# hermda02/dang

Hardware: AMD Instinct MI355X
Metric: gibbs_iterations_per_sec (higher is better)
Workload: dtype f64

## Files before the change

dang_amd/csrc/dangx_planeset.hip:

```cpp
#ifndef DX_NO_VCOEF
#define DX_VCOEF 1
#endif
#include "dx_host.h"
#include "dx_kern_planeset.h"

static int planeset_jeff(const SweepList& sl) {
    for (int q = 0; q < sl.n; ++q) if (sl.s[q].jeff) return 1;
    return 0;
}
static size_t planeset_lds(int ng, int nb, int nv, int lanes, int Sp, int jeff) {
    const int rows = nv > Sp + jeff ? nv : Sp + jeff;
    return ((size_t)(TROWS * ng + 3) * nb + (size_t)rows * (nb / lanes) * BLOCK) * sizeof(double);
}

static void item_codes(const SweepList& sl, int code[4]) {
    for (int q = 0; q < 4; ++q) code[q] = (q < sl.n) ? sl.s[q].mode + 8 * sl.s[q].pair + 16 * (sl.s[q].jeff ? 1 : 0) : 0;
}
static std::string planeset_name(int Sp, int nb, int ng, int lanes, int solve, const SweepList& sl, int bp) {
    int c[4];
    item_codes(sl, c);
    std::string s = "dxk::k_plane_set<" + std::to_string(Sp) + ", " + std::to_string(nb) + ", " + std::to_string(ng) + ", " + std::to_string(lanes) +
                    ", " + std::to_string(solve);
    for (int q = 0; q < 4; ++q) s += ", " + std::to_string(c[q]);
    return s + ", " + std::to_string(bp) + ">";
}

static int planeset_bp(dangx_ctx* ctx) {
    for (int j = 0; j < ctx->hm.nbands; ++j)
        if (ctx->hm.band[j].n != 0) return 1;
    return 0;
}

static bool planeset_builtin(int nb, int ng, int lanes, int solve, const SweepList& sl) {
    int c[4];
    item_codes(sl, c);
    if (nb == 20 && ng == 6 && lanes == 2) return solve && c[0] == CH_POW && c[1] == CH_MBB_BETA + 8 && c[2] == CH_LOGN_NUP && c[3] == 0;
    if (lanes == 1 && nb == 10 && ng == 4 && solve && sl.n == 0) return true;
    if (lanes == 1 && nb == 10 && ng == 4 && c[0] == CH_POW + 16)
        return c[1] == CH_MBB_BETA + 8 && c[2] == 0 && c[3] == 0;
    if (lanes == 1 && ((nb == 10 && ng == 4) || (solve && ((nb == 5 && ng == 3) || (nb == 3 && ng == 2)))))
        return c[0] == CH_POW && c[1] == CH_MBB_BETA + 8 && c[2] == 0 && c[3] == 0;
    return false;
}

template <int NB, int NG, int LP, int SOLVE, int C0, int C1, int C2>
// ... 39 lines not shown
    return true;
}

int dx_planeset_lanes(dangx_ctx* ctx, const GroupArgs& ga, const SweepList& sl, int solve) {
    static const bool enabled = [] { const char* e = getenv("DANGX_PLANESET"); return !(e && e[0] == '0'); }();
    static const bool small_too = [] { const char* e = getenv("DANGX_PLANESET"); return !(e && e[0] == 'p'); }();
    if (!enabled || sl.n < 0 || sl.n > 4 || (sl.n == 0 && !solve) || ga.ng < 1 || ga.ng > 6) return 0;
    static const int cap2 = [] { const char* e = getenv("DANGX_PS_CAP2"); return e ? atoi(e) : 13; }();
    const int nb = ctx->hm.nbands, Sp = sl.s2 - sl.s1 + 1, cap = (Sp == 2) ? cap2 : 16;
    for (int q = 0; q < sl.n; ++q) {
        const int m = sl.s[q].mode;
        if (m < CH_POW || m > CH_LOGN_W) return 0;
        if (sl.s[q].pair && !(m == CH_MBB_BETA || m == CH_LOGN_NUP)) return 0;
        if (sl.s[q].jeff && m != CH_POW) return 0;
    }
    FusedArgs fa;
    if (!planeset_args(ctx, ga, sl, fa)) return 0;
    if (solve && fa.cal && ga.nuc > 0) return 0;
    const int bp = planeset_bp(ctx), jf = planeset_jeff(sl);
    if (bp) {
        for (int q = 0; q < sl.n; ++q)
            if (sl.s[q].mode > CH_MBB_T || sl.s[q].jeff) return 0;
        if (!(small_too && nb <= cap && planeset_lds(ga.ng, nb, fa.nv, 1, Sp, 0) <= 80u * 1024u)) return 0;
        return dx_rtc_get(ctx, "dx_kern_planeset.h", planeset_name(Sp, nb, ga.ng, 1, solve, sl, 1)) ? 1 : 0;
    }
    int lanes = 0;
    if (small_too && nb <= cap && planeset_lds(ga.ng, nb, fa.nv, 1, Sp, jf) <= 80u * 1024u) lanes = 1;
    else if (nb > 12 && nb % 2 == 0 && nb / 2 <= cap && planeset_lds(ga.ng, nb, fa.nv, 2, Sp, jf) <= 80u * 1024u) lanes = 2;
    if (!lanes) return 0;
    if (planeset_builtin(nb, ga.ng, lanes, solve, sl)) return lanes;
    return dx_rtc_get(ctx, "dx_kern_planeset.h", planeset_name(Sp, nb, ga.ng, lanes, solve, sl, 0)) ? lanes : 0;
}

bool dx_launch_planeset(dangx_ctx* ctx, const GroupArgs& ga, const SweepList& sl, int lanes, int solve, unsigned nblk, unsigned long long* accp) {
    FusedArgs fa;
    if (lanes < 1 || lanes > 2 || !planeset_args(ctx, ga, sl, fa)) return false;
    const int nb = ctx->hm.nbands, ng = ga.ng, Sp = sl.s2 - sl.s1 + 1;
    const size_t ldsz = planeset_lds(ng, nb, fa.nv, lanes, Sp, planeset_jeff(sl));
    const int bp = planeset_bp(ctx);
    if (!bp && planeset_builtin(nb, ng, lanes, solve, sl)) {
        if (planeset_jeff(sl)) dx_launch_planeset_jeff(ctx, ga, fa, sl, Sp, solve, nblk, ldsz, accp);
        else if (nb == 20) launch_builtin<20, 6, 2, 1, CH_POW, CH_MBB_BETA + 8, CH_LOGN_NUP>(ctx, ga, fa, sl, Sp, nblk, ldsz, accp);
        else if (nb == 10 && sl.n == 0) launch_builtin<10, 4, 1, 1, 0, 0, 0>(ctx, ga, fa, sl, Sp, nblk, ldsz, accp);
        else if (nb == 10 && !solve) launch_builtin<10, 4, 1, 0, CH_POW, CH_MBB_BETA + 8, 0>(ctx, ga, fa, sl, Sp, nblk, ldsz, accp);
        else if (nb == 10) launch_builtin<10, 4, 1, 1, CH_POW, CH_MBB_BETA + 8, 0>(ctx, ga, fa, sl, Sp, nblk, ldsz, accp);
        else if (nb == 5) launch_builtin<5, 3, 1, 1, CH_POW, CH_MBB_BETA + 8, 0>(ctx, ga, fa, sl, Sp, nblk, ldsz, accp);
        else launch_builtin<3, 2, 1, 1, CH_POW, CH_MBB_BETA + 8, 0>(ctx, ga, fa, sl, Sp, nblk, ldsz, accp);
        return true;
    }
    hipFunction_t fn = dx_rtc_get(ctx, "dx_kern_planeset.h", planeset_name(Sp, nb, ng, lanes, solve, sl, bp));
    if (!fn) return false;
    const Model* dm = ctx->dm;
    GroupArgs gg = ga;
    SweepList ss = sl;
    unsigned long long* bad = ctx->counters;
    double* part = ctx->partial;
    void* args[] = {&dm, &gg, &fa, &ss, &bad, &accp, &part};
    return dx_rtc_launch(ctx, fn, nblk, ldsz, args) == 0;
}

#endif

#if defined(DX_LNL_DIAG) && !defined(DX_PS_JEFF)
extern "C" int dangx_lnl_diag(unsigned long long* out) {
    if (hipMemcpyFromSymbol(out, HIP_SYMBOL(g_lnl_diag), 2 * sizeof(unsigned long long)) != hipSuccess) return 1;
    const unsigned long long z[2] = {0ull, 0ull};
    return hipMemcpyToSymbol(HIP_SYMBOL(g_lnl_diag), z, sizeof(z)) == hipSuccess ? 0 : 1;
}
#endif
```

dang_amd/csrc/dx_args.h:

```cpp
#pragma once
#include "dx_model.h"
#include "dx_rng.h"
#include "dx_sed.h"

using namespace dx;

constexpr int BLOCK = 256;

struct GroupArgs {
    int ng;
    int gc[MAXG];
    int no;
    int oc[MAXC];
    int flag;
    int ml_mode, fluct;
    unsigned long long seed, stream;
    int nt, nglob;
    int tc[MAXT], trow[MAXT];
    int nuc, uc[MAXC];
};

__device__ __forceinline__ int flag_nplanes(int flag) { return (flag & DANGX_FLAG_QU) ? 2 : 1; }
__device__ __forceinline__ int flag_map(int flag, int p) {
    if (flag & DANGX_FLAG_QU) return 2 + p;
    if (flag & DANGX_FLAG_T) return 1;
    if (flag & DANGX_FLAG_Q) return 2;
    return 3;
}

enum { CH_GENERIC = 0, CH_POW = 1, CH_MBB_BETA = 2, CH_MBB_T = 3, CH_LOGN_NUP = 4, CH_LOGN_W = 5 };

struct IndexArgs {
    int comp, nind, s1, s2, nsample, ml_mode, mode;
    int bp;
    unsigned others;
    int jeff;
    unsigned long long seed, stream;
};

struct SweepItem {
    int comp, nind;
    int mode;
    int pair;
    int gmember;
    int jeff;
    unsigned long long stream, stream2;
};
constexpr int DX_MAX_SWEEPS = 6;
constexpr int DX_MAX_IDXSUM = 8;
struct SweepList {
    int n, nsample, ml_mode, s1, s2, pad;
    unsigned long long seed;
    SweepItem s[DX_MAX_SWEEPS];
};
```

dang_amd/csrc/dx_chain.h:

```cpp
#pragma once
#include "dx_args.h"


template <bool V> struct BoolTag { static constexpr bool value = V; };

#ifdef DX_CHAIN_LIBEXP
#define CEXP(x) exp(x)
#define CEXPS(x) exp(x)
#define CEXP1(x) exp(x)
#else
#define CEXP(x) exp_nr(x)
#define CEXPS(x) exp_sat(x)
#define CEXP1(x) exp_nr_v(x)
#endif
#ifdef DX_CHAIN_IEEEDIV
#define CDIV(a, b) ((a) / (b))
#else
#define CDIV(a, b) ((a) * fast_rcp(b))
#endif

#ifndef DX_CHAIN_UNSCALED
#define DX_CHAIN_SCALED 1
#endif
#ifndef DX_CHAIN_PAIR_RNG
// ... 18 lines not shown
}

__device__ __forceinline__ bool mh_certain(double dlo, double dhi, double u3, bool& acc) {
    const float uf = (float)u3;
    const float elo = __builtin_amdgcn_exp2f((float)dlo * 0x1.715476p+0f);
    const float ehi = __builtin_amdgcn_exp2f((float)dhi * 0x1.715476p+0f);
    acc = (dlo >= 0.0) || (elo > uf * 0x1.001p+0f);
    return acc || ((dhi < 0.0) && (ehi < uf * 0x1.ffep-1f));
}


#ifdef DX_LNL_DIAG
__device__ unsigned long long g_lnl_diag[2];
__device__ __forceinline__ void lnl_diag_count(int k) {
    if (__lane_id() == __builtin_ctzll(__builtin_amdgcn_ballot_w64(true))) atomicAdd(&g_lnl_diag[k], 1ull);
}
#endif

template <int LP>
struct BandPick {
    int half;
    __device__ __forceinline__ double operator()(const double* arr, int j, int nbh) const {
        if (LP == 1) return arr[j];
        const double a = arr[j], b = arr[nbh + j];
        return half ? b : a;
    }
    __device__ __forceinline__ double nu_c(const Model& M, int j, int nbh) const {
        if (LP == 1) return M.band[j].nu_c;
        const double a = M.band[j].nu_c, b = M.band[nbh + j].nu_c;
        return half ? b : a;
    }
};

template <int MODE, int SP, int NB, int LP, bool KT = false, bool BP = false, bool JF = false>
struct RegChain {
    static constexpr bool kBP = BP;
    static constexpr bool kJF = JF;
    static_assert(!JF || (MODE == CH_POW && !BP), "Jeffreys chains: power law, delta bands");
    double D[SP][NB], F[NB], ISr[SP][NB];
    double bpa, bpb;
    double K1[(LP > 1 && !KT) ? NB : 1], K2[(LP > 1 && !KT) ? NB : 1];
    const double *kt1, *kt2;
    double amp[SP];
    double W[(JF && !KT) ? NB : 1], jS;
    double* wcol;

    __device__ __forceinline__ double w(int j) const { return KT ? wcol[j * BLOCK] : W[j]; }
    template <class ISF>
    __device__ __forceinline__ void form_w(const Model& M, const Comp& c, ISF is_of) {
        bool bad = false;
#pragma unroll
        for (int kk = 0; kk < SP; ++kk) bad = bad || !(fabs(amp[kk]) > 0.0 && fabs(amp[kk]) < INFINITY);
#pragma unroll
        for (int j = 0; j < NB; ++j) {
            const double t0 = is_of(0, j) * is_of(0, j);
            double q = t0 * t0;
            if (SP == 2) { const double t1 = is_of(SP - 1, j) * is_of(SP - 1, j); q = fma(t1, t1, q); }
            const double l = k1(M, c, j);
            const double wj = bad ? __longlong_as_double(0x7ff8000000000000ll) : (l * l) * q;
            if (KT) wcol[j * BLOCK] = wj; else W[j] = wj;
        }
    }
    __device__ __forceinline__ void jeff_eval(const Model& M, const Comp& c, double th) {
        double S = 0.0;
#pragma unroll
        for (int j = 0; j < NB; ++j) { const double e = CEXP(th * k1(M, c, j)); S = fma(e * e, w(j), S); }
        if (LP > 1) S += __shfl_xor(S, 1, 64);
        jS = S;
    }

    __device__ __forceinline__ double is(int kk, int j) const { return ISr[kk][j]; }
    __device__ __forceinline__ void set_is(int kk, int j, double v) { ISr[kk][j] = v; }
    __device__ __forceinline__ double k1(const Model& M, const Comp& c, int j) const {
        if (KT) return kt1[j];
        if (LP > 1) return K1[j];
        return (MODE == CH_MBB_T) ? M.band[j].nu_c : (MODE == CH_LOGN_NUP) ? c.lnu9[j] : c.lnr[j];
    }
    __device__ __forceinline__ double k2(const Comp& c, int j) const { return KT ? kt2[j] : (LP > 1) ? K2[j] : c.cst[j]; }
    __device__ __forceinline__ void set_kt(const double* tab, int nbands, int ng, int g, int jb) {
        kt1 = tab + ((MODE == CH_MBB_T) ? TROWS * ng : (MODE == CH_LOGN_NUP) ? TROWS * g + 2 : TROWS * g) * nbands + jb;
        kt2 = tab + (TROWS * g + 1) * nbands + jb;
    }
    __device__ __forceinline__ void set_k(const Model& M, const Comp& c, const BandPick<LP>& pick) {
        if (LP > 1 && !KT) {
#pragma unroll
            for (int j = 0; j < NB; ++j) {
                K1[j] = (MODE == CH_MBB_T) ? pick.nu_c(M, j, NB) : (MODE == CH_LOGN_NUP) ? pick(c.lnu9, j, NB) : pick(c.lnr, j, NB);
                K2[j] = (MODE == CH_LOGN_NUP || MODE == CH_LOGN_W) ? pick(c.cst, j, NB) : 0.0;
            }
        }
    }

    template <bool BATCH, int OP = 0>
    __device__ __forceinline__ double lnl(const Model& M, const Comp& c, double th, double other, double& acc0, double& acc1) {
        double s0 = 0.0, s1 = 0.0;
        if (MODE == CH_POW) s0 = th;
        else if (MODE == CH_MBB_BETA) s0 = th + 1.0;
        else if (MODE == CH_MBB_T) { s0 = mbb_z(th); s1 = CEXP(s0 * c.nu_ref) - 1.0; }
        else if (MODE == CH_LOGN_NUP) { s0 = log_pos(th); s1 = other; }
        else s1 = th;
        acc0 = 0.0; acc1 = 0.0;
        double S = 0.0;
#ifdef DX_CHAIN_IEEEDIV
        const double rs1 = 1.0 / s1;
#else
        const double rs1 = (MODE == CH_LOGN_NUP || MODE == CH_LOGN_W) ? fast_rcp(s1) : 0.0;
#endif
        constexpr int TT = BP ? 1 : (NB % 5 == 0) ? 5 : (NB % 4 == 0) ? 4 : (NB % 3 == 0) ? 3 : 1;
        static_assert(!BP || (LP == 1 && (MODE == CH_POW || MODE == CH_MBB_BETA || MODE == CH_MBB_T)), "bandpass chains: one lane, power law / mbb");
#pragma unroll
        for (int j0 = 0; j0 < NB; j0 += TT) {
            double s[TT];
            if (BP && M.band[j0].n != 0) {
                const Band& b = M.band[j0];
                const kptr nu = as_const(M.bp_nu0 + b.off);
                const kptr tau = as_const(M.bp_tau0 + b.off);
                const kptr lnr = as_const(c.bp_lnr + b.off);
                const int n = b.n;
                double sj = 0.0;
                if (MODE == CH_POW) {
#pragma unroll 4
                    for (int q = 0; q < n; ++q) sj = sj + tau[q] * CEXP(s0 * lnr[q]);
                } else if (MODE == CH_MBB_BETA) {
#pragma unroll 4
                    for (int q = 0; q < n; ++q) sj = sj + (tau[q] * bpb) * fast_rcp(CEXP(bpa * nu[q]) - 1.0) * CEXP(s0 * lnr[q]);
                } else {
#pragma unroll 4
                    for (int q = 0; q < n; ++q) sj = sj + (tau[q] * s1) * fast_rcp(CEXP(s0 * nu[q]) - 1.0) * CEXP(bpa * lnr[q]);
                }
                s[0] = sj;
            } else
            if (MODE == CH_MBB_T && TT > 1 && BATCH) {
                double den[TT], pre[TT];
#pragma unroll
                for (int t = 0; t < TT; ++t) den[t] = CEXP(s0 * k1(M, c, j0 + t)) - 1.0;
                pre[0] = den[0];
#pragma unroll
                for (int t = 1; t < TT; ++t) pre[t] = pre[t - 1] * den[t];
                double inv = s1 * fast_rcp(pre[TT - 1]);
#pragma unroll
                for (int t = TT - 1; t > 0; --t) {
                    s[t] = (inv * pre[t - 1]) * F[j0 + t];
                    inv *= den[t];
                }
                s[0] = inv * F[j0];
            } else
#pragma unroll
            for (int t = 0; t < TT; ++t) {
                const int j = j0 + t;
                if (MODE == CH_LOGN_NUP) {
                    const double l = (k1(M, c, j) - s0) * rs1;
                    s[t] = CEXPS(-0.5 * (l * l)) * k2(c, j);
                } else if (MODE == CH_LOGN_W) {
                    const double l = F[j] * rs1;
                    s[t] = CEXPS(-0.5 * (l * l)) * k2(c, j);
                } else {
                    const double e = CEXP(s0 * k1(M, c, j));
                    if (MODE == CH_POW) s[t] = e;
                    else if (MODE == CH_MBB_BETA) s[t] = F[j] * e;
                    else s[t] = CDIV(s1, e - 1.0) * F[j];
                }
            }
#pragma unroll
            for (int t = 0; t < TT; ++t) {
                const int j = j0 + t;
#ifdef DX_CHAIN_SCALED
                if (OP == 1) {
                    const double r0 = D[0][j];
                    D[0][j] = fma(is(0, j), s[t], r0);
                    acc0 = fma(r0, r0, acc0);
                    if (SP == 2) {
                        const double r1 = D[SP - 1][j];
                        D[SP - 1][j] = fma(is(SP - 1, j), s[t], r1);
                        acc1 = fma(r1, r1, acc1);
                    }
                } else if (OP == 2) {
                    const double r0 = fma(-is(0, j), s[t], D[0][j]);
                    D[0][j] = r0;
                    acc0 = fma(r0, r0, acc0);
                    if (SP == 2) {
                        const double r1 = fma(-is(SP - 1, j), s[t], D[SP - 1][j]);
                        D[SP - 1][j] = r1;
                        acc1 = fma(r1, r1, acc1);
                    }
                } else {
                const double r0 = fma(-is(0, j), s[t], D[0][j]);
                acc0 = fma(r0, r0, acc0);
                if (SP == 2) {
                    const double r1 = fma(-is(SP - 1, j), s[t], D[SP - 1][j]);
                    acc1 = fma(r1, r1, acc1);
                }
                }
                if (JF && OP != 2) S = fma(s[t] * s[t], w(j), S);
#else
                const double r0 = (D[0][j] - amp[0] * s[t]) * is(0, j);
                acc0 = acc0 - 0.5 * (r0 * r0);
                if (SP == 2) {
                    const double r1 = (D[SP - 1][j] - amp[SP - 1] * s[t]) * is(SP - 1, j);
                    acc1 = acc1 - 0.5 * (r1 * r1);
                }
#endif
            }
        }
        if (LP > 1) {
            acc0 += __shfl_xor(acc0, 1, 64);
            if (SP == 2) acc1 += __shfl_xor(acc1, 1, 64);
            if (JF && OP != 2) S += __shfl_xor(S, 1, 64);
        }
        if (JF && OP != 2) jS = S;
#ifdef DX_CHAIN_SCALED
        acc0 *= -0.5; acc1 *= -0.5;
#endif
        return acc0 + acc1;
    }

    __device__ __forceinline__ double lnl_cheap(const Model& M, const Comp& c, double th) {
        double s0 = 0.0, s1 = 0.0;
        if (MODE == CH_POW) s0 = th;
        else if (MODE == CH_MBB_BETA) s0 = th + 1.0;
        else { s0 = mbb_z(th); s1 = CEXP(s0 * c.nu_ref) - 1.0; }
        const double s0l = s0 * 0x1.71547652b82fep+0;
        double acc0 = 0.0, acc1 = 0.0;
#pragma unroll
        for (int j = 0; j < NB; ++j) {
            const float e = __builtin_amdgcn_exp2f((float)(s0l * k1(M, c, j)));
            double s;
            if (MODE == CH_POW) s = (double)e;
            else if (MODE == CH_MBB_BETA) s = F[j] * (double)e;
            else s = (s1 * F[j]) * (double)__builtin_amdgcn_rcpf(e - 1.0f);
            const double r0 = fma(-is(0, j), s, D[0][j]);
            acc0 = fma(r0, r0, acc0);
            if (SP == 2) {
                const double r1 = fma(-is(SP - 1, j), s, D[SP - 1][j]);
                acc1 = fma(r1, r1, acc1);
            }
        }
        double a = acc0 + acc1;
        if (LP > 1) a += __shfl_xor(a, 1, 64);
        return a;
    }

    __device__ __forceinline__ bool cheap_bound(const Model& M, const Comp& c, double lo, double hi, double a_start,
                                                double& wA, double& wG) {
        double G = 0.0, emax = 0.0, kmax = 0.0;
        double smax, zmin = 0.0;
        if (MODE == CH_POW) smax = fmax(fabs(lo), fabs(hi));
        else if (MODE == CH_MBB_BETA) smax = fmax(fabs(lo + 1.0), fabs(hi + 1.0));
        else { smax = mbb_z(lo); zmin = mbb_z(hi); }
// ... 74 lines not shown
        for (int j = 0; j < NB; ++j) { const double s = CEXP(pr.p0 * pick(c2.lnr, j, NB)); Da[j] -= ampa * s; Db[j] -= ampb * s; }
        break;
    case DANGX_MBB:
#pragma unroll
        for (int j = 0; j < NB; ++j) {
            const double s = CDIV(pr.p2, CEXP(pr.p1 * pick.nu_c(M, j, NB)) - 1.0) * CEXP(pr.p0 * pick(c2.lnr, j, NB));
            Da[j] -= ampa * s; Db[j] -= ampb * s;
        }
        break;
    case DANGX_FREEFREE:
#pragma unroll
        for (int j = 0; j < NB; ++j) {
            const double s = ff_gaunt(pick(c2.lnu9, j, NB), pr.p0) / pr.p1 * pick(c2.cst, j, NB);
            Da[j] -= ampa * s; Db[j] -= ampb * s;
        }
        break;
    case DANGX_LOGNORMAL: {
        const double rp1 = fast_rcp(pr.p1);
#pragma unroll
        for (int j = 0; j < NB; ++j) {
            const double l2 = (pick(c2.lnu9, j, NB) - pr.p2) * rp1;
            const double s = CEXPS(-0.5 * (l2 * l2)) * pick(c2.cst, j, NB);
            Da[j] -= ampa * s; Db[j] -= ampb * s;
        }
        break;
    }
    default:
#pragma unroll
        for (int j = 0; j < NB; ++j) { const double s = pick(c2.cst, j, NB); Da[j] -= ampa * s; Db[j] -= ampb * s; }
        break;
    }
}

template <int MODE, int SP, int NB, int LP, bool SCALE = true, bool ADD = false, bool SUB = false, class RC>
__device__ __forceinline__ unsigned long long chain_finish(const Model& M, const IndexArgs& a, const Comp& c, RC& R,
                                                           const BandPick<LP>& pick, double sample0, double sample1, int i, int half,
                                                           double chi[4], double* final_value = nullptr,
                                                           const double* acc_in = nullptr, double* acc_out = nullptr) {
    const int npix = M.npix;
    double* out = c.idx + ((long long)a.nind * M.nmaps) * npix + i;
    const bool first = (a.nind == 0);
    constexpr bool JEFF = RC::kJF;
#if !defined(DX_CHAIN_SCALED)
    static_assert(!JEFF, "the Jeffreys chain exists in the scaled form");
#endif
    if (JEFF && SCALE) R.form_w(M, c, [&](int kk, int j) { return R.is(kk, j); });
    if (SCALE) R.scale();
    if (MODE == CH_MBB_BETA) {
        const double z = mbb_z(sample1);
        const double A = CEXP(z * c.nu_ref) - 1.0;
#pragma unroll
        for (int j = 0; j < NB; ++j) R.F[j] = CDIV(A, CEXP(z * pick.nu_c(M, j, NB)) - 1.0);
        if (RC::kBP) { R.bpa = z; R.bpb = A; }
    } else if (MODE == CH_MBB_T) {
#pragma unroll
        for (int j = 0; j < NB; ++j) R.F[j] = CEXP((sample0 + 1.0) * pick(c.lnr, j, NB));
        if (RC::kBP) R.bpa = sample0 + 1.0;
    } else if (MODE == CH_LOGN_W) {
        {
            const double lp = log_pos(sample0);
#pragma unroll
            for (int j = 0; j < NB; ++j) R.F[j] = pick(c.lnu9, j, NB) - lp;
        }
    }
    const double other = first ? sample1 : sample0;
    const unsigned long long gpix = (unsigned long long)(M.pix0 + i);
    const int q = a.nind;
    const bool gauss = c.prior_type[q] == DANGX_PRIOR_GAUSSIAN;
    const double pmean = c.gauss[q][0], pstd = c.gauss[q][1], lgden = c.lgden[q];
    const double inv2v = 1.0 / (2 * (pstd * pstd));
    auto prior = [&](double v) -> double {
        if (!gauss) return 0.0;
#ifdef DX_CHAIN_IEEEDIV
        const double arg = ((v - pmean) * (v - pmean)) / (2 * (pstd * pstd));
#else
        const double arg = ((v - pmean) * (v - pmean)) * inv2v;
#endif
        return (arg > 745.0) ? -INFINITY : -arg - lgden;
    };
    auto jprior = [&](double S) -> double {
        double p = log_pos(sqrt(S));
        if (!(S >= 0x1p-1022 && S < INFINITY)) p = log(sqrt(S));
        return p;
    };
    unsigned long long nacc = 0;
    double cur = first ? sample0 : sample1;
    double a0, a1, c0, c1;
    const double step = c.step[q], lo = c.uni[q][0], hi = c.uni[q][1];
    const bool ml_opt = (a.ml_mode == DANGX_ML_OPTIMIZE);
#if defined(DX_LNL_EXACT) || !defined(DX_CHAIN_SCALED)
    constexpr bool kCert = false;
#else
    constexpr bool kCert = !RC::kBP && !JEFF && (MODE == CH_POW || MODE == CH_MBB_BETA || MODE == CH_MBB_T);
#endif
    auto chain = [&](auto batch_tag) {
        constexpr bool B = decltype(batch_tag)::value;
        double lnl;
        if (acc_in) { a0 = acc_in[0]; a1 = acc_in[1]; lnl = a0 + a1; if (JEFF) R.jeff_eval(M, c, cur); }
        else lnl = R.template lnl<B, ADD ? 1 : 0>(M, c, cur, other, a0, a1);
        chi[0] = -2.0 * a0; chi[1] = -2.0 * a1;
        double lnl_old = lnl + (JEFF ? jprior(R.jS) : prior(cur));
        bool cert = false, old_exact = true, sums_exact = true;
        double wA = 0.0, wG = 0.0, wold = 0.0;
        if (kCert) {
            const bool ok = R.cheap_bound(M, c, lo, hi, -2.0 * lnl, wA, wG) && !ml_opt;
            cert = __builtin_amdgcn_ballot_w64(!ok) == 0ull;
        }
        auto mh_step = [&](double prop, double u3) {
            if (prop < lo || prop > hi) return;
            if constexpr (!kCert) {
                lnl = R.template lnl<B>(M, c, prop, other, c0, c1);
                const double lnl_new = lnl + (JEFF ? jprior(R.jS) : prior(prop));
                const double diff = lnl_new - lnl_old;
                const bool acc = ml_opt ? (diff > 0.0) : mh_accept(diff, u3);
                if (acc) { cur = prop; lnl_old = lnl_new; a0 = c0; a1 = c1; ++nacc; }
            } else {
                const double pp = prior(prop);
                bool acc = false, und = true;
                double lc = 0.0, wc = 0.0;
                if (cert) {
                    const double A = R.lnl_cheap(M, c, prop);
                    lc = -0.5 * A;
                    wc = fma(wA, A, wG);
                    const double dc = (lc + pp) - lnl_old;
                    const double W = (wc + wold) * (1.0 + 0x1p-40) + 0x1p-49 * ((fabs(lc) + fabs(pp)) + fabs(lnl_old));
                    und = !mh_certain(dc - W, dc + W, u3, acc);
#ifdef DX_LNL_DIAG
                    lnl_diag_count(0);
                    if (__builtin_amdgcn_ballot_w64(und) != 0ull) lnl_diag_count(1);
#endif
                }
// ... 9 lines not shown
                        }
                        const double lnl_new = lnl + pp;
                        const double diff = lnl_new - lnl_old;
                        acc = ml_opt ? (diff > 0.0) : mh_accept(diff, u3);
                        if (acc) { lnl_old = lnl_new; a0 = c0; a1 = c1; }
                        old_exact = true;
                        wold = 0.0;
                    }
                }
                if (acc) {
                    cur = prop;
                    ++nacc;
                    sums_exact = und;
                    if (!und) { lnl_old = lc + pp; wold = wc; old_exact = false; }
                }
            }
        };
        if (LP == 1 || DX_CHAIN_PAIR_RNG == 0) {
            for (int l = 1; l <= a.nsample; ++l) {
                double u1, u2, u3;
                uniform3(a.seed, a.stream, gpix, (uint32_t)l, u1, u2, u3);
                mh_step(cur + rand_normal(0.0, step, u1, u2), u3);
            }
        } else {
            for (int l = 1; l <= a.nsample; l += 2) {
                double u1, u2, u3;
                uniform3(a.seed, a.stream, gpix, (uint32_t)(l + half), u1, u2, u3);
                const double g = rand_normal(0.0, step, u1, u2);
                const double go = __shfl_xor(g, 1, 64), uo = __shfl_xor(u3, 1, 64);
                mh_step(cur + (half == 0 ? g : go), half == 0 ? u3 : uo);
                if (l + 1 <= a.nsample) mh_step(cur + (half == 0 ? go : g), half == 0 ? uo : u3);
            }
        }
        if (SUB) {
            double s0_, s1_;
            (void)R.template lnl<B, 2>(M, c, cur, other, s0_, s1_);
            if (!sums_exact) { a0 = s0_; a1 = s1_; }
        } else if (kCert) {
            if (__builtin_amdgcn_ballot_w64(!sums_exact) != 0ull) {
                if (!sums_exact) (void)R.template lnl<B>(M, c, cur, other, a0, a1);
            }
        }
    };
#ifdef DX_CHAIN_NO_BATCH_RCP
    chain(BoolTag<false>{});
#else
    if (MODE == CH_MBB_T && !RC::kBP) {
        const double tmin = fmin(lo, cur);
#ifdef DX_BATCH_ALWAYS
        chain(BoolTag<true>{});
#elif defined(DX_BATCH_LANEWISE)
        if (tmin > 0.0 && mbb_z(tmin) * M.mbb_batch_z < 1.0) chain(BoolTag<true>{});
        else chain(BoolTag<false>{});
#else
        const bool unsafe = !(tmin > 0.0 && mbb_z(tmin) * M.mbb_batch_z < 1.0);
        if (__builtin_amdgcn_ballot_w64(unsafe) == 0ull) chain(BoolTag<true>{});
        else chain(BoolTag<false>{});
#endif
    } else {
        chain(BoolTag<false>{});
    }
#endif
    if (final_value) *final_value = cur;
    if (acc_out) { acc_out[0] = a0; acc_out[1] = a1; }
    if (half != 0) {
        chi[0] = chi[1] = 0.0;
        return 0ull;
    }
#pragma unroll
// ... 121 lines not shown
```

dang_amd/csrc/dx_kern_fused.h:

```cpp
#pragma once
#include "dx_chain.h"

struct FusedArgs {
    signed char vslot[MAXG];
    signed char vcomp[MAXG];
    signed char vtype[MAXG];
    int nv;
    int gself;
    int cal;
};

#ifndef DX_FUSED_WAVES
#define DX_FUSED_WAVES(SP, NB) 2
#endif
#ifndef DX_FUSED_GRP
#define DX_FUSED_GRP 5
#endif
namespace dxk {

template <int NBL>
__device__ __forceinline__ void sed_column(int type, const double* __restrict__ tab, int NB, int NG, int g, int jb, const Prep& p,
                                           double* __restrict__ colg) {
    const double* lnr = tab + (TROWS * g) * NB + jb;
    const double* cst = lnr + NB;
    const double* lnu9 = cst + NB;
    const double* nuc = tab + (TROWS * NG) * NB + jb;
    constexpr int TT = (NBL % 5 == 0) ? 5 : (NBL % 4 == 0) ? 4 : (NBL % 3 == 0) ? 3 : 1;
    if (type == DANGX_POWERLAW) {
#pragma unroll 1
        for (int j0 = 0; j0 < NBL; j0 += TT) {
#pragma unroll
            for (int t = 0; t < TT; ++t) colg[(j0 + t) * BLOCK] = exp_nr(p.p0 * lnr[j0 + t]);
        }
    } else if (type == DANGX_MBB) {
#pragma unroll 1
        for (int j0 = 0; j0 < NBL; j0 += TT) {
            double f[TT];
#pragma unroll
            for (int t = 0; t < TT; ++t) f[t] = p.p2 * fast_rcp(exp_nr(p.p1 * nuc[j0 + t]) - 1.0);
            __builtin_amdgcn_sched_barrier(0);
#pragma unroll
            for (int t = 0; t < TT; ++t) colg[(j0 + t) * BLOCK] = f[t] * exp_nr(p.p0 * lnr[j0 + t]);
        }
    } else if (type == DANGX_FREEFREE) {
        const double rp1 = fast_rcp(p.p1);
#pragma unroll 1
        for (int j0 = 0; j0 < NBL; j0 += TT) {
#pragma unroll
            for (int t = 0; t < TT; ++t) colg[(j0 + t) * BLOCK] = (ff_gaunt(lnu9[j0 + t], p.p0) * rp1) * cst[j0 + t];
        }
    } else {
        const double rp1 = fast_rcp(p.p1);
#pragma unroll 1
        for (int j0 = 0; j0 < NBL; j0 += TT) {
#pragma unroll
            for (int t = 0; t < TT; ++t) {
                const double l = (lnu9[j0 + t] - p.p2) * rp1;
                colg[(j0 + t) * BLOCK] = exp_sat(-0.5 * (l * l)) * cst[j0 + t];
            }
        }
    }
}

template <int NBL>
__device__ __forceinline__ void sed_column_bp(const Model& M, const Comp& c2, const double* __restrict__ tab, int NB, int NG, int g,
                                              const Prep& p, double* __restrict__ colg) {
#pragma unroll 1
    for (int j = 0; j < NBL; ++j) colg[j * BLOCK] = (M.band[j].n != 0) ? sed_bandpass(M, c2, j, p) : sed_eval_tab(c2.type, tab, NB, NG, g, j, p);
}

template <int MODE, int SP, int NB, int NG, int LP, bool JF = false>
__global__ __launch_bounds__(BLOCK, DX_FUSED_WAVES(SP, NB)) void k_amp_index(const Model* __restrict__ Mp, GroupArgs ga, FusedArgs fa, IndexArgs a,
// ... 198 lines not shown
```

dang_amd/csrc/dx_kern_planeset.h:

```cpp
#pragma once
#include "dx_kern_fused.h"

#ifndef DX_PS_WAVES
#define DX_PS_WAVES(SP, NB, LP, SOLVE, C0) (((NB) / (LP) <= 5) ? 3 : 2)
#endif

namespace dxk {

template <int V> struct ItemCode { static constexpr int value = V; };
template <bool V> struct ItemFlag { static constexpr bool value = V; };

template <int MODE, int PAIR, int SP, int NBL, int LP, int NG, bool FIRST, bool LAST, bool BP, bool JF, typename RFirst>
__device__ __forceinline__ void ps_item(const Model& M, const SweepList& sl, const SweepItem& it, RFirst& R0, int i, int half,
                                        int jb, int NB, const double* __restrict__ tab, const double* __restrict__ col,
                                        double& sample0, double& sample1, double chi_first[4],
                                        double chi_last[4], unsigned int* __restrict__ accepted, int slot, const double* first_acc,
                                        double* wrow) {
    const Comp& c = M.comp[it.comp];
    const BandPick<LP> pick = {half};
    const int npix = M.npix;
    IndexArgs a;
    a.comp = it.comp; a.nind = it.nind; a.s1 = sl.s1; a.s2 = sl.s2; a.nsample = sl.nsample; a.ml_mode = sl.ml_mode; a.mode = MODE;
    a.bp = 0; a.others = 0u; a.jeff = 0; a.seed = sl.seed; a.stream = it.stream;
    RegChain<MODE, SP, NBL, LP, true, BP, JF> R;
    R.set_kt(tab, NB, NG, it.gmember, jb);
#pragma unroll
    for (int kk = 0; kk < SP; ++kk) {
        R.amp[kk] = c.amp[(long long)(sl.s1 + kk - 1) * npix + i];
#pragma unroll
        for (int j = 0; j < NBL; ++j) { R.D[kk][j] = R0.D[kk][j]; R.ISr[kk][j] = col[(kk * NBL + j) * BLOCK] * R.amp[kk]; }
    }
    if (JF) {
        R.wcol = wrow;
        R.form_w(M, c, [&](int kk, int j) { return col[(kk * NBL + j) * BLOCK]; });
    }
    double chia[4] = {0.0, 0.0, 0.0, 0.0}, va, acc[2];
    unsigned long long na = chain_finish<MODE, SP, NBL, LP, false, !FIRST, (!PAIR && !LAST)>(M, a, c, R, pick, sample0, sample1, i, half, chia, &va,
                                                                                            FIRST ? first_acc : nullptr, acc);
    if (it.nind == 0) sample0 = va; else sample1 = va;
    if (FIRST) { chi_first[0] = chia[0]; chi_first[1] = chia[1]; }
    chi_last[2] = chia[2]; chi_last[3] = chia[3];
    unsigned long long nb_ = 0ull;
    if (PAIR) {
        constexpr int MODEB = (MODE == CH_MBB_BETA || MODE == CH_LOGN_NUP) ? MODE + 1 : MODE;
        RegChain<MODEB, SP, NBL, LP, true, BP> RB;
        RB.set_kt(tab, NB, NG, it.gmember, jb);
#pragma unroll
        for (int kk = 0; kk < SP; ++kk) {
            RB.amp[kk] = R.amp[kk];
#pragma unroll
            for (int j = 0; j < NBL; ++j) { RB.D[kk][j] = R.D[kk][j]; RB.ISr[kk][j] = R.ISr[kk][j]; }
        }
        IndexArgs b = a;
        b.nind = it.nind + 1; b.stream = it.stream2; b.mode = MODEB;
        double chib[4] = {0.0, 0.0, 0.0, 0.0}, vb;
        nb_ = chain_finish<MODEB, SP, NBL, LP, false, false, !LAST>(M, b, c, RB, pick, sample0, sample1, i, half, chib, &vb, acc);
        if (b.nind == 0) sample0 = vb; else sample1 = vb;
        chi_last[2] = chib[2]; chi_last[3] = chib[3];
        if (!LAST) {
#pragma unroll
            for (int kk = 0; kk < SP; ++kk)
#pragma unroll
                for (int j = 0; j < NBL; ++j) R0.D[kk][j] = RB.D[kk][j];
        }
    } else if (!LAST) {
#pragma unroll
        for (int kk = 0; kk < SP; ++kk)
#pragma unroll
            for (int j = 0; j < NBL; ++j) R0.D[kk][j] = R.D[kk][j];
    }
    if (accepted) {
        const int copy = threadIdx.x & 15;
        if (na) atomicAdd(accepted + (slot << 4) + copy, (unsigned int)na);
        if (nb_) atomicAdd(accepted + ((slot + 1) << 4) + copy, (unsigned int)nb_);
    }
}

template <int SP, int NB, int NG, int LP, int SOLVE, int C0, int C1, int C2, int C3, int BP = 0>
__global__ __launch_bounds__(BLOCK, DX_PS_WAVES(SP, NB, LP, SOLVE, C0)) void k_plane_set(const Model* __restrict__ Mp, GroupArgs ga, FusedArgs fa, SweepList sl,
// ... 3 lines not shown
    extern __shared__ double lds[];
    const Model& M = *Mp;
    const int npix = M.npix, tid = threadIdx.x;
    double* tab = lds;
    double* col = lds + (TROWS * NG + 3) * NB + tid;
    const long long t0 = (long long)blockIdx.x * BLOCK + tid;
    const long long u = t0 / LP;
    const int half = (int)(t0 % LP), jb = half * NBL;
    const bool in_range = u < npix;
    const int i = in_range ? (int)u : 0;
    const double mk = M.mask[i];
    sed_table_build(M, tab, tid, BLOCK, ga.gc, NG);
    __shared__ unsigned int acc_blk[DX_MAX_IDXSUM * 16];
    if (tid < DX_MAX_IDXSUM * 16) acc_blk[tid] = 0u;
    __syncthreads();
    double chi[4] = {0.0, 0.0, 0.0, 0.0};
    constexpr int NS0 = C0 ? 1 + ((C0 >> 3) & 1) : 0, NS1 = C1 ? 1 + ((C1 >> 3) & 1) : 0, NS2 = C2 ? 1 + ((C2 >> 3) & 1) : 0, NS3 = C3 ? 1 + ((C3 >> 3) & 1) : 0;
    constexpr int NS = NS0 + NS1 + NS2 + NS3;
    const bool live = in_range && !is_masked(mk);
    if (in_range && !live && half == 0) {
        for (int q = 0; q < sl.n; ++q) {
            const Comp& c = M.comp[sl.s[q].comp];
            for (int e = 0; e <= sl.s[q].pair; ++e) {
                double* out = c.idx + ((long long)(sl.s[q].nind + e) * M.nmaps) * npix + i;
#pragma unroll
                for (int kk = 0; kk < SP; ++kk) out[(long long)(sl.s1 + kk - 1) * npix] = 0.0;
            }
        }
    }
    if (live) {
        const long long bstride = (long long)M.nmaps * npix;
        const unsigned long long gpix = (unsigned long long)(M.pix0 + i);
        const bool sample = (ga.ml_mode == DANGX_ML_SAMPLE);
#pragma unroll 1
        for (int v = 0; v < fa.nv; ++v) {
            const Comp& c2 = M.comp[ga.gc[fa.vcomp[v]]];
            double t0v, t1v;
            load_theta(M, c2, i, sl.s1, t0v, t1v);
            if (BP) sed_column_bp<NBL>(M, c2, tab, NB, NG, fa.vcomp[v], sed_prep(c2, t0v, t1v), col + (v * NBL) * BLOCK);
            else sed_column<NBL>(fa.vtype[v], tab, NB, NG, fa.vcomp[v], jb, sed_prep(c2, t0v, t1v), col + (v * NBL) * BLOCK);
        }
        RegChain<CH_POW, SP, NBL, LP> R0;
#pragma unroll
        for (int kk = 0; kk < SP; ++kk) {
            const int k = sl.s1 + kk;
            {
                const double* sigp = M.sig + (long long)(k - 1) * npix + i;
                const double* rmsp = M.rms + (long long)(k - 1) * npix + i;
#pragma unroll
                for (int j = 0; j < NBL; ++j) { R0.D[kk][j] = sigp[(jb + j) * bstride]; R0.ISr[kk][j] = rmsp[(jb + j) * bstride]; }
            }
            auto cal_transform = [&]() {
                const double* gn = tab + (TROWS * NG + 1) * NB + jb;
#pragma unroll
                for (int j = 0; j < NBL; ++j) R0.D[kk][j] = (R0.D[kk][j] - gn[NB + j]) / gn[j];
            };
            if (!SOLVE && SP == 1 && fa.cal) cal_transform();
#pragma unroll 1
            for (int t = 0; t < ga.nuc; ++t) {
                const Comp& ct = M.comp[ga.uc[t]];
                const double tv = ct.tmpl[(long long)(k - 1) * npix + i];
#pragma unroll
                for (int j = 0; j < NBL; ++j) R0.D[kk][j] -= ct.tamp[k - 1][jb + j] * tv;
            }
            double bv[NG];
            if (SOLVE) {
                double eta = 0.0, f0 = 0.0;
                if (sample) {
                    double u1, u2;
                    uniform2(ga.seed, ga.stream, gpix, (uint32_t)k, u1, u2);
                    eta = rand_normal(0.0, 1.0, u1, u2);
                }
                double A[NG * (NG + 1) / 2];
// ... 118 lines not shown
                const double* m = col + (fa.vslot[it0.gmember] * NBL) * BLOCK;
#pragma unroll
                for (int kk = 0; kk < SP; ++kk) {
                    const double a0 = M.comp[it0.comp].amp[(long long)(sl.s1 + kk - 1) * npix + i];
                    double acc = 0.0;
#pragma unroll
                    for (int j = 0; j < NBL; ++j) {
                        const double r = R0.D[kk][j];
                        acc = fma(r, r, acc);
                        R0.D[kk][j] = fma(a0 * R0.ISr[kk][j], m[j * BLOCK], r);
                    }
                    if (LP > 1) acc += __shfl_xor(acc, 1, 64);
                    first_acc[kk] = -0.5 * acc;
                }
            }
#pragma unroll
            for (int kk = 0; kk < SP; ++kk)
#pragma unroll
                for (int j = 0; j < NBL; ++j) col[(kk * NBL + j) * BLOCK] = R0.ISr[kk][j];
            __builtin_amdgcn_sched_barrier(0);
        }
        int slot = 0;
        auto run = [&](auto code_tag, auto first_tag, auto last_tag, int q) {
            constexpr int CODE = decltype(code_tag)::value;
            constexpr bool FIRST = decltype(first_tag)::value;
            constexpr bool LAST = decltype(last_tag)::value;
            if constexpr (CODE != 0) {
                const SweepItem it = sl.s[q];
                const Comp& c = M.comp[it.comp];
                double sample0, sample1, unused[4];
                load_theta(M, c, i, sl.s1, sample0, sample1);
                ps_item<(CODE & 7), ((CODE >> 3) & 1), SP, NBL, LP, NG, FIRST, LAST, (BP != 0), ((CODE >> 4) != 0)>(M, sl, it, R0, i, half, jb, NB, tab, col, sample0, sample1,
                                                                              FIRST ? chi : unused, chi, accepted ? acc_blk : nullptr, slot, first_acc,
                                                                              col + (SP * NBL) * BLOCK);
                slot += 1 + ((CODE >> 3) & 1);
            }
        };
        run(ItemCode<C0>{}, ItemFlag<true>{}, ItemFlag<C1 == 0>{}, 0);
        run(ItemCode<C1>{}, ItemFlag<false>{}, ItemFlag<C2 == 0>{}, 1);
        run(ItemCode<C2>{}, ItemFlag<false>{}, ItemFlag<C3 == 0>{}, 2);
        run(ItemCode<C3>{}, ItemFlag<false>{}, ItemFlag<true>{}, 3);
    }
    if (accepted && NS > 0) {
        __syncthreads();
        if (tid < NS) {
            unsigned int v = 0u;
            for (int q = 0; q < 16; ++q) v += acc_blk[(tid << 4) + q];
            if (v != 0u) atomicAdd(accepted + tid, (unsigned long long)v);
        }
    }
    if (chi_partial) {
        double isum[NS > 0 ? NS : 1];
#pragma unroll
        for (int q = 0; q < (NS > 0 ? NS : 1); ++q) isum[q] = 0.0;
        if (live && half == 0) {
            constexpr int code[4] = {C0, C1, C2, C3};
            constexpr int first[4] = {0, NS0, NS0 + NS1, NS0 + NS1 + NS2};
#pragma unroll
            for (int q = 0; q < 4; ++q)
                if (code[q] != 0) {
                    const double* at = M.comp[sl.s[q].comp].idx + ((long long)sl.s[q].nind * M.nmaps + (sl.s1 - 1)) * npix + i;
                    isum[first[q]] = at[0];
                    if (((code[q] >> 3) & 1) != 0) isum[first[q] + 1] = at[(long long)M.nmaps * npix];
                }
        }
        __shared__ double sh[4 + NS][BLOCK / 64];
#pragma unroll
// ... 16 lines not shown
```

Measured before the change: 98.80.

## Keep MBB factors from SED pass and hand exp terms between paired chains

While building the SED columns, the MBB Planck factor for the beta-sweep component is now stored in an extra LDS row, and the beta chain reads it instead of recomputing exp terms. When the chain is not first, its starting lnL is formed by adding the cached column rather than re-evaluating. At the end of the beta chain, the per-band exponentials are exported and handed to the paired temperature chain as its F factor, which skips a recompute. This costs one more LDS row per block and adds new template paths. These paths can be disabled with DX_BOUNDARY_REEVAL.

```diff
diff --git a/dang_amd/csrc/dangx_planeset.hip b/dang_amd/csrc/dangx_planeset.hip
--- a/dang_amd/csrc/dangx_planeset.hip
+++ b/dang_amd/csrc/dangx_planeset.hip
@@ -8,9 +8,25 @@
     for (int q = 0; q < sl.n; ++q) if (sl.s[q].jeff) return 1;
     return 0;
 }
-static size_t planeset_lds(int ng, int nb, int nv, int lanes, int Sp, int jeff) {
-    const int rows = nv > Sp + jeff ? nv : Sp + jeff;
+static size_t planeset_lds(int ng, int nb, int nv, int lanes, int Sp, int jeff, int keep = 0) {
+    const int rows = (nv > Sp + jeff ? nv : Sp + jeff) + (keep ? 1 : 0);
     return ((size_t)(TROWS * ng + 3) * nb + (size_t)rows * (nb / lanes) * BLOCK) * sizeof(double);
+}
+
+static int planeset_keep(const SweepList& sl, const FusedArgs& fa, int ng, int nb, int lanes, int Sp, int bp) {
+#ifdef DX_BOUNDARY_REEVAL
+    return 0;
+#else
+    if (lanes != 1 || bp || planeset_jeff(sl)) return 0;
+    const int n = sl.n < 4 ? sl.n : 4;
+    for (int q = 0; q < n; ++q) {
+        if (sl.s[q].mode != CH_MBB_BETA) continue;
+        const int v = fa.vslot[sl.s[q].gmember];
+        if (v < 0 || planeset_lds(ng, nb, fa.nv, lanes, Sp, 0, 1) > 80u * 1024u) return 0;
+        return (q > 0 && v >= Sp) ? 2 : 1;
+    }
+    return 0;
+#endif
 }
 
 static void item_codes(const SweepList& sl, int code[4]) {
@@ -116,12 +132,14 @@
     return dx_rtc_get(ctx, "dx_kern_planeset.h", planeset_name(Sp, nb, ga.ng, lanes, solve, sl, 0)) ? lanes : 0;
 }
 
-bool dx_launch_planeset(dangx_ctx* ctx, const GroupArgs& ga, const SweepList& sl, int lanes, int solve, unsigned nblk, unsigned long long* accp) {
+bool dx_launch_planeset(dangx_ctx* ctx, const GroupArgs& ga, const SweepList& sl_in, int lanes, int solve, unsigned nblk, unsigned long long* accp) {
     FusedArgs fa;
-    if (lanes < 1 || lanes > 2 || !planeset_args(ctx, ga, sl, fa)) return false;
+    if (lanes < 1 || lanes > 2 || !planeset_args(ctx, ga, sl_in, fa)) return false;
+    SweepList sl = sl_in;
     const int nb = ctx->hm.nbands, ng = ga.ng, Sp = sl.s2 - sl.s1 + 1;
-    const size_t ldsz = planeset_lds(ng, nb, fa.nv, lanes, Sp, planeset_jeff(sl));
     const int bp = planeset_bp(ctx);
+    sl.keep = planeset_keep(sl, fa, ng, nb, lanes, Sp, bp);
+    const size_t ldsz = planeset_lds(ng, nb, fa.nv, lanes, Sp, planeset_jeff(sl), sl.keep);
     if (!bp && planeset_builtin(nb, ng, lanes, solve, sl)) {
         if (planeset_jeff(sl)) dx_launch_planeset_jeff(ctx, ga, fa, sl, Sp, solve, nblk, ldsz, accp);
         else if (nb == 20) launch_builtin<20, 6, 2, 1, CH_POW, CH_MBB_BETA + 8, CH_LOGN_NUP>(ctx, ga, fa, sl, Sp, nblk, ldsz, accp);
diff --git a/dang_amd/csrc/dx_args.h b/dang_amd/csrc/dx_args.h
--- a/dang_amd/csrc/dx_args.h
+++ b/dang_amd/csrc/dx_args.h
@@ -49,7 +49,8 @@
 constexpr int DX_MAX_SWEEPS = 6;
 constexpr int DX_MAX_IDXSUM = 8;
 struct SweepList {
-    int n, nsample, ml_mode, s1, s2, pad;
+    int n, nsample, ml_mode, s1, s2;
+    int keep;
     unsigned long long seed;
     SweepItem s[DX_MAX_SWEEPS];
 };
diff --git a/dang_amd/csrc/dx_chain.h b/dang_amd/csrc/dx_chain.h
--- a/dang_amd/csrc/dx_chain.h
+++ b/dang_amd/csrc/dx_chain.h
@@ -74,10 +74,12 @@
     }
 };
 
-template <int MODE, int SP, int NB, int LP, bool KT = false, bool BP = false, bool JF = false>
+template <int MODE, int SP, int NB, int LP, bool KT = false, bool BP = false, bool JF = false, bool KEPT = false>
 struct RegChain {
     static constexpr bool kBP = BP;
     static constexpr bool kJF = JF;
+    static constexpr bool kKept = KEPT;
+    static_assert(!KEPT || (LP == 1 && !BP && !JF && (MODE == CH_MBB_BETA || MODE == CH_MBB_T)), "kept factors: one-lane delta-band mbb chains");
     static_assert(!JF || (MODE == CH_POW && !BP), "Jeffreys chains: power law, delta bands");
     double D[SP][NB], F[NB], ISr[SP][NB];
     double bpa, bpb;
@@ -86,6 +88,7 @@
     double amp[SP];
     double W[(JF && !KT) ? NB : 1], jS;
     double* wcol;
+    const double* fcol;
 
     __device__ __forceinline__ double w(int j) const { return KT ? wcol[j * BLOCK] : W[j]; }
     template <class ISF>
@@ -133,8 +136,10 @@
         }
     }
 
-    template <bool BATCH, int OP = 0>
-    __device__ __forceinline__ double lnl(const Model& M, const Comp& c, double th, double other, double& acc0, double& acc1) {
+    template <bool BATCH, int OP = 0, bool EOUT = false>
+    __device__ __forceinline__ double lnl(const Model& M, const Comp& c, double th, double other, double& acc0, double& acc1,
+                                          double* eout = nullptr) {
+        static_assert(!EOUT || (MODE == CH_MBB_BETA && !BP), "the exported factor is the beta chain's");
         double s0 = 0.0, s1 = 0.0;
         if (MODE == CH_POW) s0 = th;
         else if (MODE == CH_MBB_BETA) s0 = th + 1.0;
@@ -198,6 +203,7 @@
                     s[t] = CEXPS(-0.5 * (l * l)) * k2(c, j);
                 } else {
                     const double e = CEXP(s0 * k1(M, c, j));
+                    if (EOUT) eout[j] = e;
                     if (MODE == CH_POW) s[t] = e;
                     else if (MODE == CH_MBB_BETA) s[t] = F[j] * e;
                     else s[t] = CDIV(s1, e - 1.0) * F[j];
@@ -256,6 +262,25 @@
         return acc0 + acc1;
     }
 
+    __device__ __forceinline__ double lnl_add_kept(const double* scol, double& acc0, double& acc1) {
+        static_assert(LP == 1 && !JF && !BP, "one lane, delta bands, no prior sum");
+        acc0 = 0.0; acc1 = 0.0;
+#pragma unroll
+        for (int j = 0; j < NB; ++j) {
+            const double s = scol[j * BLOCK];
+            const double r0 = D[0][j];
+            D[0][j] = fma(is(0, j), s, r0);
+            acc0 = fma(r0, r0, acc0);
+            if (SP == 2) {
+                const double r1 = D[SP - 1][j];
+                D[SP - 1][j] = fma(is(SP - 1, j), s, r1);
+                acc1 = fma(r1, r1, acc1);
+            }
+        }
+        acc0 *= -0.5; acc1 *= -0.5;
+        return acc0 + acc1;
+    }
+
     __device__ __forceinline__ double lnl_cheap(const Model& M, const Comp& c, double th) {
         double s0 = 0.0, s1 = 0.0;
         if (MODE == CH_POW) s0 = th;
@@ -396,11 +421,13 @@
     }
 }
 
-template <int MODE, int SP, int NB, int LP, bool SCALE = true, bool ADD = false, bool SUB = false, class RC>
+template <int MODE, int SP, int NB, int LP, bool SCALE = true, bool ADD = false, bool SUB = false, bool HAND = false, class RC>
 __device__ __forceinline__ unsigned long long chain_finish(const Model& M, const IndexArgs& a, const Comp& c, RC& R,
                                                            const BandPick<LP>& pick, double sample0, double sample1, int i, int half,
                                                            double chi[4], double* final_value = nullptr,
-                                                           const double* acc_in = nullptr, double* acc_out = nullptr) {
+                                                           const double* acc_in = nullptr, double* acc_out = nullptr,
+                                                           double* hand = nullptr, const double* scol = nullptr) {
+    static_assert(!HAND || (MODE == CH_MBB_BETA && !SUB && !RC::kBP && LP == 1), "the hand-over is the one-lane delta-band beta chain's");
     const int npix = M.npix;
     double* out = c.idx + ((long long)a.nind * M.nmaps) * npix + i;
     const bool first = (a.nind == 0);
@@ -410,7 +437,11 @@
 #endif
     if (JEFF && SCALE) R.form_w(M, c, [&](int kk, int j) { return R.is(kk, j); });
     if (SCALE) R.scale();
-    if (MODE == CH_MBB_BETA) {
+    if (MODE == CH_MBB_BETA && RC::kKept && R.fcol) {
+#pragma unroll
+        for (int j = 0; j < NB; ++j) R.F[j] = R.fcol[j * BLOCK];
+    } else if (MODE == CH_MBB_T && RC::kKept) {
+    } else if (MODE == CH_MBB_BETA) {
         const double z = mbb_z(sample1);
         const double A = CEXP(z * c.nu_ref) - 1.0;
 #pragma unroll
@@ -461,6 +492,10 @@
         constexpr bool B = decltype(batch_tag)::value;
         double lnl;
         if (acc_in) { a0 = acc_in[0]; a1 = acc_in[1]; lnl = a0 + a1; if (JEFF) R.jeff_eval(M, c, cur); }
+        else if constexpr (ADD && RC::kKept) {
+            if (scol) lnl = R.lnl_add_kept(scol, a0, a1);
+            else lnl = R.template lnl<B, 1>(M, c, cur, other, a0, a1);
+        }
         else lnl = R.template lnl<B, ADD ? 1 : 0>(M, c, cur, other, a0, a1);
         chi[0] = -2.0 * a0; chi[1] = -2.0 * a1;
         double lnl_old = lnl + (JEFF ? jprior(R.jS) : prior(cur));
@@ -536,9 +571,13 @@
                 if (l + 1 <= a.nsample) mh_step(cur + (half == 0 ? go : g), half == 0 ? uo : u3);
             }
         }
-        if (SUB) {
+        if constexpr (SUB) {
             double s0_, s1_;
             (void)R.template lnl<B, 2>(M, c, cur, other, s0_, s1_);
+            if (!sums_exact) { a0 = s0_; a1 = s1_; }
+        } else if constexpr (HAND) {
+            double s0_, s1_;
+            (void)R.template lnl<B, 0, true>(M, c, cur, other, s0_, s1_, hand);
             if (!sums_exact) { a0 = s0_; a1 = s1_; }
         } else if (kCert) {
             if (__builtin_amdgcn_ballot_w64(!sums_exact) != 0ull) {
diff --git a/dang_amd/csrc/dx_kern_fused.h b/dang_amd/csrc/dx_kern_fused.h
--- a/dang_amd/csrc/dx_kern_fused.h
+++ b/dang_amd/csrc/dx_kern_fused.h
@@ -20,7 +20,7 @@
 
 template <int NBL>
 __device__ __forceinline__ void sed_column(int type, const double* __restrict__ tab, int NB, int NG, int g, int jb, const Prep& p,
-                                           double* __restrict__ colg) {
+                                           double* __restrict__ colg, double* __restrict__ fcol = nullptr) {
     const double* lnr = tab + (TROWS * g) * NB + jb;
     const double* cst = lnr + NB;
     const double* lnu9 = cst + NB;
@@ -38,6 +38,10 @@
             double f[TT];
 #pragma unroll
             for (int t = 0; t < TT; ++t) f[t] = p.p2 * fast_rcp(exp_nr(p.p1 * nuc[j0 + t]) - 1.0);
+            if (fcol) {
+#pragma unroll
+                for (int t = 0; t < TT; ++t) fcol[(j0 + t) * BLOCK] = f[t];
+            }
             __builtin_amdgcn_sched_barrier(0);
 #pragma unroll
             for (int t = 0; t < TT; ++t) colg[(j0 + t) * BLOCK] = f[t] * exp_nr(p.p0 * lnr[j0 + t]);
diff --git a/dang_amd/csrc/dx_kern_planeset.h b/dang_amd/csrc/dx_kern_planeset.h
--- a/dang_amd/csrc/dx_kern_planeset.h
+++ b/dang_amd/csrc/dx_kern_planeset.h
@@ -10,20 +10,27 @@
 template <int V> struct ItemCode { static constexpr int value = V; };
 template <bool V> struct ItemFlag { static constexpr bool value = V; };
 
+#ifdef DX_BOUNDARY_REEVAL
+#define DX_PS_SHARE(MODE, LP, BP, JF) false
+#else
+#define DX_PS_SHARE(MODE, LP, BP, JF) ((MODE) == CH_MBB_BETA && (LP) == 1 && !(BP) && !(JF))
+#endif
 template <int MODE, int PAIR, int SP, int NBL, int LP, int NG, bool FIRST, bool LAST, bool BP, bool JF, typename RFirst>
 __device__ __forceinline__ void ps_item(const Model& M, const SweepList& sl, const SweepItem& it, RFirst& R0, int i, int half,
                                         int jb, int NB, const double* __restrict__ tab, const double* __restrict__ col,
                                         double& sample0, double& sample1, double chi_first[4],
                                         double chi_last[4], unsigned int* __restrict__ accepted, int slot, const double* first_acc,
-                                        double* wrow) {
+                                        double* wrow, const double* fkeep, const double* skeep) {
     const Comp& c = M.comp[it.comp];
     const BandPick<LP> pick = {half};
     const int npix = M.npix;
     IndexArgs a;
     a.comp = it.comp; a.nind = it.nind; a.s1 = sl.s1; a.s2 = sl.s2; a.nsample = sl.nsample; a.ml_mode = sl.ml_mode; a.mode = MODE;
     a.bp = 0; a.others = 0u; a.jeff = 0; a.seed = sl.seed; a.stream = it.stream;
-    RegChain<MODE, SP, NBL, LP, true, BP, JF> R;
+    constexpr bool SHARE = DX_PS_SHARE(MODE, LP, BP, JF);
+    RegChain<MODE, SP, NBL, LP, true, BP, JF, SHARE> R;
     R.set_kt(tab, NB, NG, it.gmember, jb);
+    R.fcol = fkeep;
 #pragma unroll
     for (int kk = 0; kk < SP; ++kk) {
         R.amp[kk] = c.amp[(long long)(sl.s1 + kk - 1) * npix + i];
@@ -35,16 +42,22 @@
         R.form_w(M, c, [&](int kk, int j) { return col[(kk * NBL + j) * BLOCK]; });
     }
     double chia[4] = {0.0, 0.0, 0.0, 0.0}, va, acc[2];
-    unsigned long long na = chain_finish<MODE, SP, NBL, LP, false, !FIRST, (!PAIR && !LAST)>(M, a, c, R, pick, sample0, sample1, i, half, chia, &va,
-                                                                                            FIRST ? first_acc : nullptr, acc);
+    constexpr bool HAND = SHARE && PAIR != 0;
+    double ej[HAND ? NBL : 1];
+    unsigned long long na = chain_finish<MODE, SP, NBL, LP, false, !FIRST, (!PAIR && !LAST), HAND>(M, a, c, R, pick, sample0, sample1, i, half, chia, &va,
+                                                                                                  FIRST ? first_acc : nullptr, acc, ej, skeep);
     if (it.nind == 0) sample0 = va; else sample1 = va;
     if (FIRST) { chi_first[0] = chia[0]; chi_first[1] = chia[1]; }
     chi_last[2] = chia[2]; chi_last[3] = chia[3];
     unsigned long long nb_ = 0ull;
     if (PAIR) {
         constexpr int MODEB = (MODE == CH_MBB_BETA || MODE == CH_LOGN_NUP) ? MODE + 1 : MODE;
-        RegChain<MODEB, SP, NBL, LP, true, BP> RB;
+        RegChain<MODEB, SP, NBL, LP, true, BP, false, HAND> RB;
         RB.set_kt(tab, NB, NG, it.gmember, jb);
+        if (HAND) {
+#pragma unroll
+            for (int j = 0; j < NBL; ++j) RB.F[j] = ej[j];
+        }
 #pragma unroll
         for (int kk = 0; kk < SP; ++kk) {
             RB.amp[kk] = R.amp[kk];
@@ -114,13 +127,20 @@
         const long long bstride = (long long)M.nmaps * npix;
         const unsigned long long gpix = (unsigned long long)(M.pix0 + i);
         const bool sample = (ga.ml_mode == DANGX_ML_SAMPLE);
+        constexpr int KQ = ((C0 & 7) == CH_MBB_BETA) ? 0 : ((C1 & 7) == CH_MBB_BETA) ? 1 : ((C2 & 7) == CH_MBB_BETA) ? 2 : 3;
+        constexpr bool KEEPC = DX_PS_SHARE(CH_MBB_BETA, LP, BP, false) &&
+                               ((C0 & 7) == CH_MBB_BETA || (C1 & 7) == CH_MBB_BETA || (C2 & 7) == CH_MBB_BETA || (C3 & 7) == CH_MBB_BETA);
+        const int kv = (KEEPC && sl.keep > 0) ? fa.vslot[sl.s[KQ].gmember] : -1;
+        double* const fkeep = (kv >= 0) ? col + ((fa.nv > SP ? fa.nv : SP) * NBL) * BLOCK : nullptr;
+        const double* const skeep = (kv >= 0 && sl.keep == 2) ? col + (kv * NBL) * BLOCK : nullptr;
 #pragma unroll 1
         for (int v = 0; v < fa.nv; ++v) {
             const Comp& c2 = M.comp[ga.gc[fa.vcomp[v]]];
             double t0v, t1v;
             load_theta(M, c2, i, sl.s1, t0v, t1v);
             if (BP) sed_column_bp<NBL>(M, c2, tab, NB, NG, fa.vcomp[v], sed_prep(c2, t0v, t1v), col + (v * NBL) * BLOCK);
-            else sed_column<NBL>(fa.vtype[v], tab, NB, NG, fa.vcomp[v], jb, sed_prep(c2, t0v, t1v), col + (v * NBL) * BLOCK);
+            else sed_column<NBL>(fa.vtype[v], tab, NB, NG, fa.vcomp[v], jb, sed_prep(c2, t0v, t1v), col + (v * NBL) * BLOCK,
+                                 (KEEPC && v == kv) ? fkeep : nullptr);
         }
         RegChain<CH_POW, SP, NBL, LP> R0;
 #pragma unroll
@@ -305,7 +325,8 @@
                 load_theta(M, c, i, sl.s1, sample0, sample1);
                 ps_item<(CODE & 7), ((CODE >> 3) & 1), SP, NBL, LP, NG, FIRST, LAST, (BP != 0), ((CODE >> 4) != 0)>(M, sl, it, R0, i, half, jb, NB, tab, col, sample0, sample1,
                                                                               FIRST ? chi : unused, chi, accepted ? acc_blk : nullptr, slot, first_acc,
-                                                                              col + (SP * NBL) * BLOCK);
+                                                                              col + (SP * NBL) * BLOCK, (KEEPC && q == KQ) ? fkeep : nullptr,
+                                                                              (KEEPC && q == KQ) ? skeep : nullptr);
                 slot += 1 + ((CODE >> 3) & 1);
             }
         };
```

Measured after the change: 100.7, median of 6. 1.9% higher.
